# VITA-Group/Open-L2O

Measured on NVIDIA H100. Metric: coordinate-updates/sec (N_params x unroll_steps), higher is better.
Workload: dtype f32

## Files before the change

### open_l2o_b200/csrc/cwlstm_tc_bwd.cuh

```cuda
#pragma once
#include "cwlstm_tc.cuh"

namespace l2o {
namespace tcb {

using namespace tc;

constexpr int kBwdWG = 2;
constexpr int kBwdThreads = 128 * kBwdWG;
constexpr uint32_t kXaLBO = 8 * 128;
constexpr uint32_t kXbLBO = 10 * 128;
constexpr uint32_t kXaBytes = 8 * kXaLBO;
constexpr uint32_t kXbBytes = 8 * kXbLBO;
constexpr int kBlkL1 = 5, kRowOne2 = 63;

__device__ __forceinline__ void split_bf16x2(float v0, float v1, uint32_t& hi, uint32_t& lo) {
  asm("cvt.rn.bf16x2.f32 %0, %1, %2;" : "=r"(hi) : "f"(v1), "f"(v0));
  const float r0 = v0 - __uint_as_float(hi << 16), r1 = v1 - __uint_as_float(hi & 0xFFFF0000u);
  asm("cvt.rn.bf16x2.f32 %0, %1, %2;" : "=r"(lo) : "f"(r1), "f"(r0));
}
__device__ __forceinline__ void stsm_x4_trans(uint32_t sa, uint32_t r0, uint32_t r1, uint32_t r2, uint32_t r3) {
  asm volatile("stmatrix.sync.aligned.m8n8.x4.trans.shared.b16 [%0], {%1, %2, %3, %4};" ::"r"(sa), "r"(r0), "r"(r1),
               "r"(r2), "r"(r3)
               : "memory");
}
__device__ __forceinline__ void mma_ss_bf16_n80(float* d, uint64_t a, uint64_t b) {
  asm volatile(
      "{\n\t.reg .pred p;\n\tsetp.ne.b32 p, %42, 0;\n\t"
      "wgmma.mma_async.sync.aligned.m64n80k16.f32.bf16.bf16 "
      "{%0,%1,%2,%3,%4,%5,%6,%7,%8,%9,%10,%11,%12,%13,%14,%15,%16,%17,%18,%19,"
      "%20,%21,%22,%23,%24,%25,%26,%27,%28,%29,%30,%31,%32,%33,%34,%35,%36,%37,%38,%39}, "
      "%40, %41, p, 1, 1, 0, 0;\n\t}\n"
      : L2O_ACC8(0), L2O_ACC8(8), L2O_ACC8(16), L2O_ACC8(24), L2O_ACC8(32)
      : "l"(a), "l"(b), "r"(1));
}
__device__ __forceinline__ void wg_bar(int wg) { asm volatile("bar.sync %0, 128;" ::"r"(1 + wg) : "memory"); }
__device__ __forceinline__ void prefetch_l2_bulk(const void* p, uint32_t bytes) {
  asm volatile("cp.async.bulk.prefetch.L2.global [%0], %1;" ::"l"(p), "r"(bytes) : "memory");
}
__device__ __forceinline__ void prefetch_l2(const void* p) { asm volatile("prefetch.global.L2 [%0];" ::"l"(p)); }

__device__ __forceinline__ void unit_bwd(float& zi, float& zj, float& zf, float& zo, float cprev, float dh, float& dc, float& hn) {
  const float i = sigmoid_fast(zi), j = tanh_fast(zj), f = sigmoid_fast(zf + 1.0f), o = sigmoid_fast(zo);
  const float cn = fmaf(f, cprev, i * j);
  const float tcn = tanh_fast(cn);
  hn = tcn * o;
  const float dho = dh * o;
  const float dcv = fmaf(dho, fmaf(-tcn, tcn, 1.0f), dc);
  zi = (dcv * j) * fmaf(-i, i, i);
  zj = (dcv * i) * fmaf(-j, j, 1.0f);
  zf = (dcv * cprev) * fmaf(-f, f, f);
  zo = (dho * tcn) * (1.0f - o);
  dc = dcv * f;
}

template <class C, int MODE>
__device__ __forceinline__ int dw_row(int m) {
  const int p = (m & 7) >> 1, slot = 2 * (m >> 3) + (m & 1);
  if (m == kRowOne2) return MODE == 2 ? C::O_B1 : C::O_B2;
  if (slot < 2 * kBlkL1) {
    const int u = 5 * p + slot % kU;
    if (MODE == 2) return C::O_W1 + (slot < kU ? C::F + u : u) * C::G1;
    return C::O_W2 + (slot < kU ? u : kH + u) * C::G2;
  }
  if (MODE == 0) {
    const int s = slot - 2 * kBlkL1;
    if (s < kU) return C::O_W1 + (C::F + 5 * p + s) * C::G1;
    if (p < C::F) return C::O_W1 + p * C::G1;
    if (p == C::F) return C::O_B1;
  }
  return -1;
}

template <class C, int MODE>
struct SmemB {
  float img[Geo<C>::AllFloats];
  float wo[kH + 4];
  float win[64];
  uint64_t wbar, pad;
};
template <class C, int MODE>
__host__ __device__ constexpr uint32_t stage_bytes() {
  return (MODE == 0 ? 4 : 2) * kXaBytes + 2 * kXbBytes;
}
struct alignas(16) CkRing {
  float h[tc::kTile * kH], c2[tc::kTile * kH], c1[tc::kTile * kH];
  uint64_t barh, bar2, bar1;
};
template <class C, int MODE>
__host__ __device__ constexpr size_t bwd_smem_bytes() {
  return ((sizeof(SmemB<C, MODE>) + 1023) & ~(size_t)1023) +
         (size_t)kBwdWG * (stage_bytes<C, MODE>() + (MODE == 0 ? sizeof(CkRing) : 0));
}

template <class C, int MODE>
__global__ void __launch_bounds__(kBwdThreads, 1) unroll_bwd_kernel(l2o_bwd_args a, NetRt rt, const float* __restrict__ img) {
  using G = Geo<C>;
  static_assert(MODE == 0 ? !C::FC : C::FC, "DM nets: one pass; fc nets: two passes");
  static_assert(MODE != 0 || C::F < 3, "the feature chunk leaves quad thread 3's slot of row 63 to layer 2's 1");
  extern __shared__ __align__(1024) unsigned char smem_raw[];
  SmemB<C, MODE>& S = *reinterpret_cast<SmemB<C, MODE>*>(smem_raw);
  const int wg = threadIdx.x >> 7, warp = (threadIdx.x >> 5) & 3, lane = threadIdx.x & 31;
  const int g = lane >> 2, q = lane & 3;
  const uint32_t stage = smem_u32(smem_raw) + (uint32_t)((sizeof(SmemB<C, MODE>) + 1023) & ~(size_t)1023) +
                         (uint32_t)wg * stage_bytes<C, MODE>();
  constexpr uint32_t kXa2 = 0, kXa1 = 2 * kXaBytes;
  constexpr uint32_t kXb = (MODE == 0 ? 4 : 2) * kXaBytes;
  constexpr bool kL2 = MODE != 2, kL1 = MODE != 1;
  constexpr bool kRing = MODE == 0;
  CkRing& R = *reinterpret_cast<CkRing*>(smem_raw + ((sizeof(SmemB<C, MODE>) + 1023) & ~(size_t)1023) +
                                         (size_t)kBwdWG * stage_bytes<C, MODE>() + (size_t)wg * sizeof(CkRing));
  const bool elected = (threadIdx.x & 127) == 0;

  for (uint32_t o = threadIdx.x * 4; o < kBwdWG * stage_bytes<C, MODE>(); o += blockDim.x * 4) {
    const uint32_t ow = o % stage_bytes<C, MODE>();
    const uint32_t v = (ow < kXaBytes && (ow % kXaLBO) >> 4 == (uint32_t)kRowOne2) ? 0x3F803F80u : 0u;
    asm volatile("st.shared.u32 [%0], %1;" ::"r"(stage - (uint32_t)wg * stage_bytes<C, MODE>() + o), "r"(v) : "memory");
  }
  if (threadIdx.x < kH) S.wo[threadIdx.x] = a.theta[C::O_WO + threadIdx.x];
  if constexpr (C::FC) {
    if (threadIdx.x >= 32 && threadIdx.x < 92) S.win[threadIdx.x - 32] = a.theta[C::O_WIN + threadIdx.x - 32];
  }
  if (threadIdx.x == 0) {
    mbar_init(&S.wbar, 1);
    if (!kRing) fence_barrier_init();
  }
  if (kRing && elected) {
    mbar_init(&R.barh, 1);
    mbar_init(&R.bar2, 1);
    mbar_init(&R.bar1, 1);
    fence_barrier_init();
  }
  fence_proxy_async();
  __syncthreads();
  stage_image(S.img, img, G::AllFloats * 4, &S.wbar);

  const uint64_t b1h = img_desc(S.img, kN), b1l = img_desc(S.img + G::B1Floats, kN);
  const uint64_t b2h = img_desc(S.img + 2 * G::B1Floats, kN), b2l = img_desc(S.img + 2 * G::B1Floats + G::B2Floats, kN);
  const float* tbase = S.img + G::FwdFloats;
  const uint64_t t1h = img_desc(tbase, G::N1), t1l = img_desc(tbase + G::T1Floats, G::N1);
  const uint64_t t2h = img_desc(tbase + 2 * G::T1Floats, G::N2), t2l = img_desc(tbase + 2 * G::T1Floats + G::T2Floats, G::N2);
  const uint64_t xbh = make_desc(stage + kXb, kXbLBO, 128), xbl = make_desc(stage + kXb + kXbBytes, kXbLBO, 128);
  const uint64_t xa2h = make_desc(stage + kXa2, kXaLBO, 128), xa2l = make_desc(stage + kXa2 + kXaBytes, kXaLBO, 128);
  const uint64_t xa1h = make_desc(stage + (MODE == 0 ? kXa1 : kXa2), kXaLBO, 128);
  const uint64_t xa1l = make_desc(stage + (MODE == 0 ? kXa1 : kXa2) + kXaBytes, kXaLBO, 128);

  const int T = a.T;
  const int64_t n = a.n, slot = n * C::SF;
  const int64_t ntiles = (n + tc::kTile - 1) / tc::kTile;
  const bool imit = a.labels != nullptr;
  const float inv_nt = imit ? 1.0f / (float)a.n_total : 0.f;
  float wo[kU];
#pragma unroll
  for (int s = 0; s < kU; ++s) wo[s] = S.wo[5 * q + s];
  float acc_wo[kU] = {0.f, 0.f, 0.f, 0.f, 0.f}, acc_bo = 0.f;
  float aw0[kU] = {0.f, 0.f, 0.f, 0.f, 0.f}, aw1[kU] = {0.f, 0.f, 0.f, 0.f, 0.f}, ab[kU] = {0.f, 0.f, 0.f, 0.f, 0.f};
  float dw[kN / 2];
#pragma unroll
  for (int k = 0; k < kN / 2; ++k) dw[k] = 0.f;
  const int kx = warp * 16 + g;
  const int64_t tstride = (int64_t)gridDim.x * kBwdWG;

  auto ck_block = [&](int64_t tl, int t, int blk) {
    return a.ckpt + (int64_t)t * slot + (blk * n + tl * tc::kTile) * kH;
  };
  auto tile_bytes = [&](int64_t tl) {
    const int64_t r = n - tl * tc::kTile;
    return (uint32_t)((r < tc::kTile ? r : tc::kTile) * kH * 4);
  };
  auto arm = [&](uint64_t* bar, float* dst, int64_t tl, int t, int blk) {
    const uint32_t b = tile_bytes(tl);
    mbar_expect_tx(bar, b);
    tma_bulk_g2s(dst, ck_block(tl, t, blk), b, bar);
  };
  auto ring5 = [&](const float* buf, int rh, bool on, float* v) {
    const float* p = buf + (kx + 8 * rh) * kH + 5 * q;
#pragma unroll
    for (int s = 0; s < kU; ++s) v[s] = on ? p[s] : 0.f;
  };
  if constexpr (kRing) {
    const int64_t tile0 = (int64_t)blockIdx.x * kBwdWG + wg;
    if (elected && tile0 < ntiles) {
      arm(&R.barh, R.h, tile0, T - 1, 2);
      arm(&R.bar2, R.c2, tile0, T - 1, 3);
      arm(&R.bar1, R.c1, tile0, T - 1, 1);
    }
  }
  uint32_t ph = 0;

  Frag<G::KB> A;
  const int blk = lane >> 3;
  const uint32_t la = stage + (uint32_t)((2 * warp + (blk & 1)) * (int)kXaLBO + (blk >> 1) * (int)kXaBytes + (lane & 7) * 16);
  const uint32_t lb = stage + kXb + (uint32_t)((2 * warp + (blk & 1)) * (int)kXbLBO + (blk >> 1) * (int)kXbBytes + (lane & 7) * 16);
  auto stage_x = [&](uint32_t buf, int b0, int nb, int c0, int c1) {
    auto val = [&](int i, int rh) { return A.get_at(i < kU ? c0 + 4 * i : c1 + 4 * (i - kU), rh); };
#pragma unroll
    for (int b = 0; b < nb; ++b) {
      uint32_t h0, l0, h1, l1;
      split_bf16x2(val(2 * b, 0), val(2 * b + 1, 0), h0, l0);
      split_bf16x2(val(2 * b, 1), val(2 * b + 1, 1), h1, l1);
      stsm_x4_trans(la + buf + (uint32_t)(b0 + b) * 128, h0, h1, l0, l1);
    }
  };
  auto stage_dz = [&](const float* z) {
#pragma unroll
    for (int j = 0; j < kN / 8; ++j) {
      uint32_t h0, l0, h1, l1;
      split_bf16x2(z[4 * j], z[4 * j + 1], h0, l0);
      split_bf16x2(z[4 * j + 2], z[4 * j + 3], h1, l1);
      stsm_x4_trans(lb + (uint32_t)j * 128, h0, h1, l0, l1);
    }
  };
  auto dx_dw = [&](auto ncols, float* z, float* x, uint64_t th, uint64_t tl, uint64_t xah, uint64_t xal) {
    constexpr int NX = decltype(ncols)::value;
    uint32_t fh[kN / 8][4], fl[kN / 8][4];
#pragma unroll
    for (int j = 0; j < kN / 8; ++j) {
      split_tf32(z[4 * j + 0], fh[j][0], fl[j][0]);
      split_tf32(z[4 * j + 2], fh[j][1], fl[j][1]);
      split_tf32(z[4 * j + 1], fh[j][2], fl[j][2]);
      split_tf32(z[4 * j + 3], fh[j][3], fl[j][3]);
    }
    constexpr uint64_t step = img_kstep(NX);
    wg_fence();
#pragma unroll
    for (int j = 0; j < kN / 8; ++j) {
      mma_rs<NX>(x, fl[j], th + j * step, j > 0 ? 1u : 0u);
      mma_rs<NX>(x, fh[j], tl + j * step, 1u);
      mma_rs<NX>(x, fh[j], th + j * step, 1u);
    }
    wg_commit();
    constexpr uint64_t sa = (2 * kXaLBO) >> 4, sb = (2 * kXbLBO) >> 4;
#pragma unroll
    for (int kk = 0; kk < tc::kTile / 16; ++kk) {
      mma_ss_bf16_n80(dw, xal + kk * sa, xbh + kk * sb);
      mma_ss_bf16_n80(dw, xah + kk * sa, xbl + kk * sb);
      mma_ss_bf16_n80(dw, xah + kk * sa, xbh + kk * sb);
    }
    wg_commit();
    wg_wait<1>();
  };
  auto flush_dw = [&]() {
    wg_wait<0>();
#pragma unroll
    for (int rh = 0; rh < 2; ++rh) {
      const int r = dw_row<C, MODE>(kx + 8 * rh);
#pragma unroll
      for (int j = 0; j < kN / 8; ++j)
#pragma unroll
        for (int e = 0; e < 2; ++e) {
          float& v = dw[4 * j + 2 * rh + e];
          if (r >= 0 && v != 0.f) atomicAdd(&a.dtheta[r + gate_ref_col(8 * j + 2 * q + e)], (double)v);
          v = 0.f;
        }
    }
  };

  for (int64_t tile = (int64_t)blockIdx.x * kBwdWG + wg; tile < ntiles; tile += tstride) {
    const int64_t r0 = tile * tc::kTile + warp * 16 + g;
    const int64_t row[2] = {r0, r0 + 8};
    const bool act[2] = {row[0] < n, row[1] < n};
    float dc2[2][kU], dh2c[2][kU], dc1[2][kU], dh1c[2][kU];
#pragma unroll
    for (int rh = 0; rh < 2; ++rh)
#pragma unroll
      for (int s = 0; s < kU; ++s) { dc2[rh][s] = 0.f; dh2c[rh][s] = 0.f; dc1[rh][s] = 0.f; dh1c[rh][s] = 0.f; }
    float lam[2];
#pragma unroll
    for (int rh = 0; rh < 2; ++rh) lam[rh] = (kL2 && act[rh] && !imit) ? a.g_rec[(int64_t)T * n + row[rh]] : 0.f;
    A.zero();
    A.template put<(G::ColOne & ~3)>(0, q == (G::ColOne & 3) ? 1.0f : 0.f);
    A.template put<(G::ColOne & ~3)>(1, q == (G::ColOne & 3) ? 1.0f : 0.f);

    for (int t = T - 1; t >= 0; --t) {
      const float* ck = a.ckpt + (int64_t)t * slot;
      const int64_t tl_next = t > 0 ? tile : tile + tstride;
      const int t_next = t > 0 ? t - 1 : T - 1;
      float z[kN / 2];
      float dh1n[2][kU];
      if constexpr (kL2) {
        float c2p[2][kU], dy[2];
        if constexpr (kRing) mbar_wait(&R.barh, 0);
#pragma unroll
        for (int rh = 0; rh < 2; ++rh) {
          float h1n[kU] = {0.f, 0.f, 0.f, 0.f, 0.f}, h2p[kU] = {0.f, 0.f, 0.f, 0.f, 0.f};
#pragma unroll
          for (int s = 0; s < kU; ++s) c2p[rh][s] = 0.f;
          float dtanh = 1.0f;
          if (act[rh]) {
            const int64_t i = row[rh];
            if constexpr (kRing) {
              if (t == T - 1) load5(ck + slot + i * kH, q, h1n);
              ring5(R.h, rh, true, h2p);
            } else {
              load5(ck + slot + i * kH, q, h1n);
              load5(ck + 2 * n * kH + i * kH, q, h2p);
              load5(ck + 2 * n * kH + (n + i) * kH, q, c2p[rh]);
            }
            if (imit) lam[rh] = (a.delta_seq[(int64_t)t * n + i] - a.labels[(int64_t)t * n + i]) * inv_nt;
            if (rt.tanh_output) {
              const float th = a.delta_seq[(int64_t)t * n + i] / rt.scale;
              dtanh = fmaf(-th, th, 1.0f);
            }
          }
          dy[rh] = rt.scale * lam[rh] * dtanh;
          if (!kRing || t == T - 1) A.template put_vec<G::ColH1>(rh, h1n);
          A.template put_vec<G::ColH2>(rh, h2p);
        }
        wg_fence();
        mma3<kN, G::KB, G::L2Lo, G::L2Hi>(z, A, b2h, b2l);
        wg_commit();
        wg_wait<0>();
        if constexpr (kRing) {
          mbar_wait(&R.bar2, ph);
#pragma unroll
          for (int rh = 0; rh < 2; ++rh) ring5(R.c2, rh, act[rh], c2p[rh]);
        }
        if (q == 0) acc_bo += dy[0] + dy[1];
#pragma unroll
        for (int rh = 0; rh < 2; ++rh)
#pragma unroll
          for (int s = 0; s < kU; ++s) {
            float hn;
            unit_bwd(z[acc_idx(s, 0, rh)], z[acc_idx(s, 1, rh)], z[acc_idx(s, 2, rh)], z[acc_idx(s, 3, rh)], c2p[rh][s],
                     fmaf(wo[s], dy[rh], dh2c[rh][s]), dc2[rh][s], hn);
            acc_wo[s] = fmaf(hn, dy[rh], acc_wo[s]);
          }
        wg_bar(wg);
        if (kRing && elected) {
          arm(&R.barh, R.h, tile, t, 0);
          if (tl_next < ntiles) arm(&R.bar2, R.c2, tl_next, t_next, 3);
        }
        stage_x(kXa2, 0, kBlkL1, G::ColH1, G::ColH2);
        stage_dz(z);
        fence_proxy_async();
        wg_bar(wg);
        float x2[G::N2 / 2];
        dx_dw(IC<G::N2>{}, z, x2, t2h, t2l, xa2h, xa2l);
#pragma unroll
        for (int rh = 0; rh < 2; ++rh)
#pragma unroll
          for (int s = 0; s < kU; ++s) {
            dh1n[rh][s] = x2[4 * (s >> 1) + 2 * rh + (s & 1)];
            dh2c[rh][s] = x2[4 * (3 + (s >> 1)) + 2 * rh + (s & 1)];
          }
        if constexpr (MODE == 1) {
#pragma unroll
          for (int rh = 0; rh < 2; ++rh)
            if (act[rh]) store5(a.scratch + ((int64_t)t * n + row[rh]) * kH, q, dh1n[rh]);
        }
#pragma unroll
        for (int rh = 0; rh < 2; ++rh)
          if (!imit && act[rh]) lam[rh] += a.g_rec[(int64_t)t * n + row[rh]];
      }
      if constexpr (kL1) {
        float c1p[2][kU];
        float r0v[2] = {0.f, 0.f}, r1v[2] = {0.f, 0.f};
        float ep[2][kU];
        if constexpr (kRing) mbar_wait(&R.barh, 1);
#pragma unroll
        for (int rh = 0; rh < 2; ++rh) {
          float h1p[kU] = {0.f, 0.f, 0.f, 0.f, 0.f};
#pragma unroll
          for (int s = 0; s < kU; ++s) c1p[rh][s] = 0.f;
          if (act[rh]) {
            const int64_t i = row[rh];
            if constexpr (kRing) {
              ring5(R.h, rh, true, h1p);
            } else {
              load5(ck + i * kH, q, h1p);
              load5(ck + (n + i) * kH, q, c1p[rh]);
            }
            if constexpr (MODE == 2) {
              load5(a.scratch + ((int64_t)t * n + i) * kH, q, dh1n[rh]);
              r0v[rh] = a.in_seq[((int64_t)t * 2) * n + i];
              r1v[rh] = a.in_seq[((int64_t)t * 2 + 1) * n + i];
            } else {
              r0v[rh] = a.in_seq[(int64_t)t * n + i];
            }
          } else if constexpr (MODE == 2) {
#pragma unroll
            for (int s = 0; s < kU; ++s) dh1n[rh][s] = 0.f;
          }
          A.template put_vec<G::ColH1>(rh, h1p);
          if constexpr (MODE == 2) {
            float e[kU];
#pragma unroll
            for (int s = 0; s < kU; ++s) {
              const int u = 5 * q + s;
              const float av = fmaf(r1v[rh], S.win[kH + u], fmaf(r0v[rh], S.win[u], S.win[2 * kH + u]));
              e[s] = elu_fast(av);
              ep[rh][s] = av > 0.f ? 1.0f : e[s] + 1.0f;
            }
            A.template put_vec<0>(rh, e);
          } else {
            float f[C::F];
            preprocess<C>(nullptr, rt, r0v[rh], 0.f, f);
            float v = q == C::F ? 1.0f : 0.f;
#pragma unroll
            for (int k = 0; k < C::F; ++k)
              if (q == k) v = f[k];
            A.template put<0>(rh, v);
          }
        }
        wg_fence();
        mma3<kN, G::KB, G::L1Lo, G::L1Hi>(z, A, b1h, b1l);
        wg_commit();
        wg_wait<0>();
        if constexpr (kRing) {
          mbar_wait(&R.bar1, ph);
#pragma unroll
          for (int rh = 0; rh < 2; ++rh) ring5(R.c1, rh, act[rh], c1p[rh]);
        }
#pragma unroll
        for (int rh = 0; rh < 2; ++rh)
#pragma unroll
          for (int s = 0; s < kU; ++s) {
            float hn;
            unit_bwd(z[acc_idx(s, 0, rh)], z[acc_idx(s, 1, rh)], z[acc_idx(s, 2, rh)], z[acc_idx(s, 3, rh)], c1p[rh][s],
                     dh1c[rh][s] + dh1n[rh][s], dc1[rh][s], hn);
          }
        wg_bar(wg);
        if constexpr (kRing) {
          if (elected && tl_next < ntiles) {
            arm(&R.barh, R.h, tl_next, t_next, 2);
            arm(&R.bar1, R.c1, tl_next, t_next, 1);
            prefetch_l2_bulk(ck_block(tl_next, t_next, 0), tile_bytes(tl_next));
          }
#pragma unroll
          for (int rh = 0; rh < 2; ++rh) {
            const int64_t r = tl_next * tc::kTile + kx + 8 * rh;
            if (q == 0 && r < n) prefetch_l2(a.in_seq + (int64_t)t_next * n + r);
          }
          ph ^= 1u;
        }
        if constexpr (MODE == 2) stage_x(kXa2, 0, kBlkL1, G::ColH1, 0);
        else stage_x(kXa1, kBlkL1, 3, G::ColH1, 0);
        stage_dz(z);
        fence_proxy_async();
        wg_bar(wg);
        float x1[G::N1 / 2];
        dx_dw(IC<G::N1>{}, z, x1, t1h, t1l, xa1h, xa1l);
#pragma unroll
        for (int rh = 0; rh < 2; ++rh)
#pragma unroll
          for (int s = 0; s < kU; ++s) {
            dh1c[rh][s] = x1[4 * (s >> 1) + 2 * rh + (s & 1)];
            if constexpr (MODE == 2) {
              const float da = x1[4 * (3 + (s >> 1)) + 2 * rh + (s & 1)] * ep[rh][s];
              aw0[s] = fmaf(r0v[rh], da, aw0[s]);
              aw1[s] = fmaf(r1v[rh], da, aw1[s]);
              ab[s] += da;
            }
          }
      }
    }
    flush_dw();
  }
  wg_wait<0>();
  auto red8 = [&](float v) {
#pragma unroll
    for (int o = 4; o < 32; o <<= 1) v += __shfl_xor_sync(0xffffffffu, v, o);
    return v;
  };
#pragma unroll
  for (int s = 0; s < kU; ++s) {
    const int u = 5 * q + s;
    if constexpr (kL2) {
      const float v = red8(acc_wo[s]);
      if (lane < 4) atomicAdd(&a.dtheta[C::O_WO + u], (double)v);
    }
    if constexpr (MODE == 2) {
      const float v0 = red8(aw0[s]), v1 = red8(aw1[s]), vb = red8(ab[s]);
      if (lane < 4) {
        atomicAdd(&a.dtheta[C::O_WIN + u], (double)v0);
        atomicAdd(&a.dtheta[C::O_WIN + C::F + u], (double)v1);
        atomicAdd(&a.dtheta[C::O_BIN + u], (double)vb);
      }
    }
  }
  if constexpr (kL2) {
    const float v = red8(acc_bo);
    if (lane == 0) atomicAdd(&a.dtheta[C::O_BO], (double)v);
  }
}

}

template <class C>
int tc_launch_bwd(const NetRt& rt, const l2o_bwd_args& a, float* img, cudaStream_t st, int sms, bool prep = true) {
  if (prep) tc::prep_weights_kernel<C><<<16, 256, 0, st>>>(a.theta, img, 1);
  const int64_t ntiles = (a.n + tc::kTile - 1) / tc::kTile;
  const int64_t ctas = (ntiles + tcb::kBwdWG - 1) / tcb::kBwdWG;
  const int grid = (int)(ctas < sms ? ctas : sms);
  auto launch = [&](auto kern, size_t smem) {
    if (smem > 227 * 1024) return L2O_E_INVALID;
    if (cudaFuncSetAttribute(kern, cudaFuncAttributeMaxDynamicSharedMemorySize, (int)smem) != cudaSuccess) return L2O_E_CUDA;
    kern<<<grid, tcb::kBwdThreads, smem, st>>>(a, rt, img);
    return cudaGetLastError() == cudaSuccess ? L2O_OK : L2O_E_CUDA;
  };
  if constexpr (C::FC) {
    int rc = launch(tcb::unroll_bwd_kernel<C, 1>, tcb::bwd_smem_bytes<C, 1>());
    if (rc != L2O_OK) return rc;
    return launch(tcb::unroll_bwd_kernel<C, 2>, tcb::bwd_smem_bytes<C, 2>());
  } else {
    return launch(tcb::unroll_bwd_kernel<C, 0>, tcb::bwd_smem_bytes<C, 0>());
  }
}

}
```

Baseline: 1.726 billion.

## Defer trailing dW wgmma chunks to overlap with next gate GEMM

In the fc-net backward modes, only the first two k-chunks of the dW wgmma are issued right after the dx GEMM. The remaining chunks are issued while waiting on the next gate GEMM, so tensor-core work on dW overlaps with the z accumulation instead of being drained with a full wait. A zeroed dz stage at the end of each tile keeps the leftover deferred MMAs harmless. The tile loop is also specialised for full tiles so the row-bounds checks become compile-time true. This adds wait and sync complexity, and depends on the deferred operand buffers (always the xa1 pair) still holding the right data when those MMAs run.

```diff
diff --git a/open_l2o_b200/csrc/cwlstm_tc_bwd.cuh b/open_l2o_b200/csrc/cwlstm_tc_bwd.cuh
--- a/open_l2o_b200/csrc/cwlstm_tc_bwd.cuh
+++ b/open_l2o_b200/csrc/cwlstm_tc_bwd.cuh
@@ -107,6 +107,8 @@
   constexpr uint32_t kXa2 = 0, kXa1 = 2 * kXaBytes;
   constexpr uint32_t kXb = (MODE == 0 ? 4 : 2) * kXaBytes;
   constexpr bool kL2 = MODE != 2, kL1 = MODE != 1;
+  constexpr bool kSplitDw = MODE != 0;
+  constexpr int kDwAfterDx = kSplitDw ? 2 : tc::kTile / 16;
   constexpr bool kRing = MODE == 0;
   CkRing& R = *reinterpret_cast<CkRing*>(smem_raw + ((sizeof(SmemB<C, MODE>) + 1023) & ~(size_t)1023) +
                                          (size_t)kBwdWG * stage_bytes<C, MODE>() + (size_t)wg * sizeof(CkRing));
@@ -211,6 +213,15 @@
       stsm_x4_trans(lb + (uint32_t)j * 128, h0, h1, l0, l1);
     }
   };
+  auto dw_mma = [&](uint64_t xah, uint64_t xal, int k0, int k1) {
+    constexpr uint64_t sa = (2 * kXaLBO) >> 4, sb = (2 * kXbLBO) >> 4;
+#pragma unroll
+    for (int kk = k0; kk < k1; ++kk) {
+      mma_ss_bf16_n80(dw, xal + kk * sa, xbh + kk * sb);
+      mma_ss_bf16_n80(dw, xah + kk * sa, xbl + kk * sb);
+      mma_ss_bf16_n80(dw, xah + kk * sa, xbh + kk * sb);
+    }
+  };
   auto dx_dw = [&](auto ncols, float* z, float* x, uint64_t th, uint64_t tl, uint64_t xah, uint64_t xal) {
     constexpr int NX = decltype(ncols)::value;
     uint32_t fh[kN / 8][4], fl[kN / 8][4];
@@ -230,15 +241,18 @@
       mma_rs<NX>(x, fh[j], th + j * step, 1u);
     }
     wg_commit();
-    constexpr uint64_t sa = (2 * kXaLBO) >> 4, sb = (2 * kXbLBO) >> 4;
-#pragma unroll
-    for (int kk = 0; kk < tc::kTile / 16; ++kk) {
-      mma_ss_bf16_n80(dw, xal + kk * sa, xbh + kk * sb);
-      mma_ss_bf16_n80(dw, xah + kk * sa, xbl + kk * sb);
-      mma_ss_bf16_n80(dw, xah + kk * sa, xbh + kk * sb);
-    }
+    dw_mma(xah, xal, 0, kDwAfterDx);
     wg_commit();
     wg_wait<1>();
+  };
+  auto z_wait = [&]() {
+    if constexpr (kSplitDw) {
+      dw_mma(xa1h, xa1l, kDwAfterDx, tc::kTile / 16);
+      wg_commit();
+      wg_wait<1>();
+    } else {
+      wg_wait<0>();
+    }
   };
   auto flush_dw = [&]() {
     wg_wait<0>();
@@ -256,10 +270,11 @@
     }
   };
 
-  for (int64_t tile = (int64_t)blockIdx.x * kBwdWG + wg; tile < ntiles; tile += tstride) {
+  auto tile_body = [&](int64_t tile, auto full_c) {
+    constexpr bool full = decltype(full_c)::value != 0;
     const int64_t r0 = tile * tc::kTile + warp * 16 + g;
     const int64_t row[2] = {r0, r0 + 8};
-    const bool act[2] = {row[0] < n, row[1] < n};
+    const bool act[2] = {full || row[0] < n, full || row[1] < n};
     float dc2[2][kU], dh2c[2][kU], dc1[2][kU], dh1c[2][kU];
 #pragma unroll
     for (int rh = 0; rh < 2; ++rh)
@@ -310,7 +325,7 @@
         wg_fence();
         mma3<kN, G::KB, G::L2Lo, G::L2Hi>(z, A, b2h, b2l);
         wg_commit();
-        wg_wait<0>();
+        z_wait();
         if constexpr (kRing) {
           mbar_wait(&R.bar2, ph);
 #pragma unroll
@@ -326,6 +341,7 @@
                      fmaf(wo[s], dy[rh], dh2c[rh][s]), dc2[rh][s], hn);
             acc_wo[s] = fmaf(hn, dy[rh], acc_wo[s]);
           }
+        if constexpr (kSplitDw) wg_wait<0>();
         wg_bar(wg);
         if (kRing && elected) {
           arm(&R.barh, R.h, tile, t, 0);
@@ -406,7 +422,7 @@
         wg_fence();
         mma3<kN, G::KB, G::L1Lo, G::L1Hi>(z, A, b1h, b1l);
         wg_commit();
-        wg_wait<0>();
+        z_wait();
         if constexpr (kRing) {
           mbar_wait(&R.bar1, ph);
 #pragma unroll
@@ -420,6 +436,7 @@
             unit_bwd(z[acc_idx(s, 0, rh)], z[acc_idx(s, 1, rh)], z[acc_idx(s, 2, rh)], z[acc_idx(s, 3, rh)], c1p[rh][s],
                      dh1c[rh][s] + dh1n[rh][s], dc1[rh][s], hn);
           }
+        if constexpr (kSplitDw) wg_wait<0>();
         wg_bar(wg);
         if constexpr (kRing) {
           if (elected && tl_next < ntiles) {
@@ -455,7 +472,23 @@
           }
       }
     }
+    if constexpr (kSplitDw) {
+      wg_fence();
+      dw_mma(xa1h, xa1l, kDwAfterDx, tc::kTile / 16);
+      wg_commit();
+    }
     flush_dw();
+    if constexpr (kSplitDw) {
+      wg_bar(wg);
+      const float zero[kN / 2] = {};
+      stage_dz(zero);
+      fence_proxy_async();
+      wg_bar(wg);
+    }
+  };
+  for (int64_t tile = (int64_t)blockIdx.x * kBwdWG + wg; tile < ntiles; tile += tstride) {
+    if (MODE != 2 && (tile + 1) * tc::kTile <= n) tile_body(tile, IC<MODE != 2>{});
+    else tile_body(tile, IC<0>{});
   }
   wg_wait<0>();
   auto red8 = [&](float v) {
```

Result: faster. 1.760 billion (median of 6 runs) (+2.0%).
